# stevenmiller888/mlx-audio

Measured on AMD Instinct MI355X. Metric: audio-sec/sec (xRT), Kokoro-82M batch=32 fixed 128-phoneme utterances per GPU, higher is better.
Workload: dtype bf16; 1 GPU; Kokoro-82M bf16, batch=32/GPU fixed 128-phoneme utterances (T=130, F=650, 390000 samples = 16.25 s each), utterance-sharded over 1 GPU(s); global_batch=32, parallelism=utterance-shard x1, 2 batches in flight per GPU

## Files before the change

include/kokoro_hip.h:

```cpp
#ifndef KOKORO_HIP_H
#define KOKORO_HIP_H

#include <stddef.h>
#include <stdint.h>

#ifdef __cplusplus
extern "C" {
#endif

#define KK_ABI_VERSION 2
#define KK_ABI_MINOR 14

enum { KK_DTYPE_F32 = 0, KK_DTYPE_BF16 = 1, KK_DTYPE_I32 = 2, KK_DTYPE_F16 = 3 };
enum { KK_NOISE_ZERO = 0, KK_NOISE_INJECTED = 1, KK_NOISE_PHILOX = 2 };

typedef struct kk_model kk_model;
typedef struct kk_context kk_context;

typedef struct kk_config {
  int32_t n_token, hidden_dim, style_dim, n_layer, max_dur, text_encoder_kernel_size;
  int32_t plbert_hidden, plbert_heads, plbert_intermediate, plbert_max_pos, plbert_layers, plbert_embedding;
  int32_t decoder_hidden;
  int32_t upsample_initial_channel;
  int32_t n_upsamples;
// ... 56 lines not shown
int kk_op_adain(void* stream, int B, const void* x, int ldx, int L_rows, const int32_t* len, int C, const float* gamma_beta, int gbs,
                int act, float slope, const float* alpha, int pool, const float* pool_w, const float* pool_b, void* out, int ldo, int Cpad,
                int Lout_rows, float* scratch, size_t scratch_floats, int dtype, int fast);
int kk_op_layernorm(void* stream, int B, const void* x, int ldx, const void* res, int ldr, int L_rows, const int32_t* len, int C,
                    const float* w, const float* b, const float* gamma_beta, int gbs, float eps, int act, float slope, void* out, int ldo,
                    int dtype);
int kk_op_lstm(void* stream, int B, const float* xproj, const float* whT, int H, int L_rows, const int32_t* len, void* out, int ldo,
               int dtype);
int kk_op_linear_rows(void* stream, int B, const void* x_bf16, long long xbs, int ldx, int rows, const int32_t* len, const void* w_bf16, int N, int K,
                      const float* bias, int act, void* pack_scratch, void* out_bf16, long long obs, int ldo);
int kk_op_lstm_bf16(void* stream, int B, const float* xproj, const void* wh_bf16, int L_rows, const int32_t* len, void* out, int ldo,
                    int dtype);
int kk_op_attention(void* stream, int B, const void* qkv, int ld, int T_rows, const int32_t* len, int heads, void* out, int ldo, int dtype);
int kk_op_source_stft(void* stream, int B, const float* f0, int L2_rows, const int32_t* len2, const float* lin_w9, float lin_b,
                      int noise_mode, const float* noise, uint64_t seed, float* phase_scratch, float* har_source, void* har, int ldhar,
                      int dtype);
int kk_op_istft_head(void* stream, int B, const void* x, int ldx, int Tf_rows, const int32_t* len_frames, float* wav, int dtype, int fast);
int kk_op_pack_head_w(void* stream, const void* w_bf16, void* w_frag);
int kk_op_conv_post_istft(void* stream, int B, const void* x, int ldx, int Tf_rows, const int32_t* len_frames, const void* w_frag,
                          const float* bias, float in_slope, float* wav, void* cp_out, int cp_ld);

int kk_mxfp8_bytes(int rows, int K, size_t* q_bytes, size_t* s_bytes);
int kk_mxfp8_pack_weight(const float* w_host, int N, int K, int group, uint8_t* q_host, uint8_t* s_host);
int kk_op_linear_mxfp8(void* stream, const void* x_bf16, int ldx, int M, int rows_per_item, const int32_t* len, int K, const void* wq,
                       const void* ws, int N, const float* bias, int act, void* aq, void* as, void* out_bf16, int ldo);

int kk_debug_info(kk_context* cx, const char* name, int64_t* rows, int64_t* channels);
int kk_debug_fetch(kk_context* cx, void* stream, const char* name, float* dst);
int kk_debug_override(kk_context* cx, const char* name, const float* src);
void kk_debug_clear(kk_context* cx);
int kk_op_pack_w_frag(void* stream, const void* w_bf16, void* w_frag, int Kw, int CoutP, int CinP);
void kk_debug_set_op_wfrag(const void* w_frag);
void kk_debug_set_op_variant(int v);
void kk_debug_set_op_post_slope(float slope);
void kk_debug_force_generic(kk_context* cx, int flags);

int kk_profile_begin(kk_context* cx, int max_launches);
int kk_profile_end(kk_context* cx, int ncls, double* ms, double* flops, double* bytes, int64_t* count);

typedef struct kk_mimi kk_mimi;

typedef struct kk_mimi_config {
  int32_t dim, nq, bins, qdim, num_heads, num_layers, dim_feedforward, nfilters;
  int32_t n_ratios, ratios[8];
  int32_t ksize, residual_ksize, last_ksize, upsample_stride, compress;
  float rope_base;
  int32_t compute_dtype;
} kk_mimi_config;

int kk_mimi_create(const kk_mimi_config* cfg, kk_mimi** out);
void kk_mimi_destroy(kk_mimi* m);
int kk_mimi_load_tensor(kk_mimi* m, const char* name, const int64_t* shape, int ndim, const float* data);
int kk_mimi_finalize(kk_mimi* m, void* stream);
int64_t kk_mimi_samples_per_frame(const kk_mimi* m);
size_t kk_mimi_workspace_bytes(kk_mimi* m, int B, int Nf);
int kk_mimi_decode(kk_mimi* m, void* stream, int B, int Nf, const int32_t* codes, void* workspace, size_t workspace_bytes, float* pcm_out);
int kk_mimi_encode_frames(const kk_mimi* m, int N);
size_t kk_mimi_encode_workspace_bytes(kk_mimi* m, int B, int N);
int kk_mimi_encode(kk_mimi* m, void* stream, int B, int N, const float* pcm, void* workspace, size_t workspace_bytes, int32_t* codes_out);
typedef struct kk_mimi_stream kk_mimi_stream;
int kk_mimi_stream_create(kk_mimi* m, int max_batch, int max_frames, kk_mimi_stream** out);
int kk_mimi_stream_create_chunked(kk_mimi* m, int encoder, int max_batch, int max_frames, int chunk_frames, kk_mimi_stream** out);
void kk_mimi_stream_destroy(kk_mimi_stream* s);
int kk_mimi_stream_reset(kk_mimi_stream* s);
int kk_mimi_stream_frames(const kk_mimi_stream* s);
int kk_mimi_stream_chunk_frames(const kk_mimi_stream* s);
// ... 169 lines not shown
```

mlx-audio_amd/_lib.py:

```python
from __future__ import annotations

import ctypes as C
import os

_HERE = os.path.dirname(os.path.abspath(__file__))
LIB_PATH = os.path.join(_HERE, "libkokoro_hip.so")

KK_F32, KK_BF16, KK_I32, KK_F16 = 0, 1, 2, 3
CSM_WEIGHTS = {0: "f32", 1: "bf16", 2: "q8", 3: "q4"}
CSM_WEIGHTS_MIXED, CSM_WEIGHTS_DEQUANTIZED = 0x100, 0x200
NOISE_ZERO, NOISE_INJECTED, NOISE_PHILOX = 0, 1, 2
ACT_NONE, ACT_LRELU, ACT_GELU, ACT_SNAKE = 0, 1, 2, 3
KK_PCM_F32, KK_PCM_S16LE, KK_PCM_MULAW, KK_PCM_ALAW = 0, 1, 2, 3


class KKConfig(C.Structure):
    _fields_ = [
        ("n_token", C.c_int32), ("hidden_dim", C.c_int32), ("style_dim", C.c_int32), ("n_layer", C.c_int32),
        ("max_dur", C.c_int32), ("text_encoder_kernel_size", C.c_int32),
        ("plbert_hidden", C.c_int32), ("plbert_heads", C.c_int32), ("plbert_intermediate", C.c_int32),
        ("plbert_max_pos", C.c_int32), ("plbert_layers", C.c_int32), ("plbert_embedding", C.c_int32),
        ("decoder_hidden", C.c_int32), ("upsample_initial_channel", C.c_int32), ("n_upsamples", C.c_int32),
        ("upsample_rates", C.c_int32 * 4), ("upsample_kernel_sizes", C.c_int32 * 4),
        ("n_resblock_kernels", C.c_int32), ("resblock_kernel_sizes", C.c_int32 * 4),
# ... 153 lines not shown
    "kk_resampler_destroy": (None, [_vp]),
    "kk_resampler_set_row": (_i, [_vp, _vp, _i, _i, _i, _vp, _i]),
    "kk_resampler_step": (_i, [_vp, _vp, _vp, C.c_longlong, _vp, _vp, _vp, C.c_longlong, _vp]),
    "kk_resampler_block_outputs": (_i, []),
    "kk_op_resample": (_i, [_vp, _vp, _i, _i, _i, _vp, _i, _vp]),
    "kk_resampler_set_row_fmt": (_i, [_vp, _vp, _i, _i, _i, _vp, _i, _i, _i]),
    "kk_resampler_step_fmt": (_i, [_vp, _vp, _vp, C.c_longlong, _vp, _vp, _vp, C.c_longlong, _vp]),
    "kk_pcm_convert_rows": (_i, [_vp, _i, _vp, C.c_longlong, _vp, _vp, C.c_longlong, _vp, _vp]),
    "kk_op_pcm_convert": (_i, [_vp, _vp, _i, _vp, _i, _i]),
    "kk_vad_create": (_i, [_i, C.POINTER(_vp)]),
    "kk_vad_destroy": (None, [_vp]),
    "kk_vad_set_row": (_i, [_vp, _vp, _i, _i, _f, _i]),
    "kk_vad_step": (_i, [_vp, _vp, _vp, C.c_longlong, _vp, _vp, _vp, C.c_longlong]),
    "kk_op_vad": (_i, [_vp, _vp, _i, _i, _f, _i, _vp, _vp]),
    "kk_vad_ring_create": (_i, [_i, C.POINTER(_vp)]),
    "kk_vad_ring_destroy": (None, [_vp]),
    "kk_vad_ring_set_row": (_i, [_vp, _vp, _i, _i, _f, _i, C.c_longlong, C.c_longlong]),
    "kk_vad_ring_step": (_i, [_vp, _vp, _vp, C.c_longlong, _vp, _vp, _vp, _vp, _vp, C.c_longlong]),
    "kk_ring_write_rows": (_i, [_vp, _i, _vp, C.c_longlong, _vp, C.c_longlong, C.c_longlong, _vp, _vp]),
    "kk_ring_read_rows": (_i, [_vp, _i, _vp, C.c_longlong, C.c_longlong, _vp, C.c_longlong, _vp, _vp, _vp]),
    "kk_op_log_mel": (_i, [_vp, _i, _vp, C.c_longlong, _vp, _i, _i, _vp, _vp, _vp, _vp, _vp, _i]),
    "kk_op_attention_long": (_i, [_vp, _i, _vp, _i, _i, _i, _i, _vp, _i]),
    "kk_whisper_create": (_i, [C.POINTER(KKWhisperConfig), C.POINTER(_vp)]),
    "kk_whisper_destroy": (None, [_vp]),
    "kk_whisper_load_tensor": (_i, [_vp, C.c_char_p, C.POINTER(C.c_int64), _i, _vp]),
    "kk_whisper_finalize": (_i, [_vp, _vp]),
    "kk_whisper_encode_workspace_bytes": (_sz, [_vp, _i]),
    "kk_whisper_encode": (_i, [_vp, _vp, _i, _vp, _vp, _sz, _vp]),
    "kk_mimi_debug_info": (_i, [_vp, C.c_char_p, C.POINTER(C.c_int64), C.POINTER(C.c_int64)]),
    "kk_mimi_debug_fetch": (_i, [_vp, _vp, C.c_char_p, _vp]),
    "kk_debug_set_op_wfrag": (None, [_vp]),
    "kk_debug_set_op_variant": (None, [_i]),
    "kk_debug_set_op_post_slope": (None, [_f]),
    "kk_set_graph_mode": (_i, [_vp, _i]),
    "kk_set_quantization": (_i, [_vp, _i, _i]),
    "kk_quantized_layers": (_i, [_vp]),
    "kk_mxfp8_bytes": (_i, [_i, _i, C.POINTER(_sz), C.POINTER(_sz)]),
    "kk_mxfp8_pack_weight": (_i, [_vp, _i, _i, _i, _vp, _vp]),
    "kk_op_linear_mxfp8": (_i, [_vp, _vp, _i, _i, _i, _vp, _i, _vp, _vp, _i, _vp, _i, _vp, _vp, _vp, _i]),
    "kk_profile_begin": (_i, [_vp, _i]),
    "kk_profile_end": (_i, [_vp, _i, C.POINTER(C.c_double), C.POINTER(C.c_double), C.POINTER(C.c_double), C.POINTER(C.c_int64)]),
}

_lib = None


class KokoroHipError(RuntimeError):
    pass


def load():
    global _lib
    if _lib is not None:
        return _lib
    path = os.environ.get("KK_HIP_LIB", LIB_PATH)
    if not os.path.exists(path):
        raise KokoroHipError(
            f"{path} not found: build it with `python mlx-audio_amd/build.py` (hipcc, gfx950). "
            "The Kokoro hot path has no CPU or PyTorch fallback."
        )
    try:
        import torch
    except ImportError:
        pass
    lib = C.CDLL(path)
    for name, (res, args) in SIGNATURES.items():
# ... 14 lines not shown
```

mlx-audio_amd/csrc/kk_conv_mfma4.hip:

```cpp
#include <stdlib.h>

#include "kk_common.h"
#include "kk_kernels.h"
#include "kk_conv_mfma_shared.h"

#define TR_NOW() 0ull
#define TR_ADD(slot, v) do { } while (0)
namespace {
typedef __bf16 bf16x2 __attribute__((ext_vector_type(2)));

typedef __bf16 bf16x8 __attribute__((ext_vector_type(8)));
typedef float f32x4 __attribute__((ext_vector_type(4)));

constexpr int BN = 128, CK = 64;
constexpr int XLD = 80;
constexpr int MAX_HALO = 50;
constexpr int CLD = BN;

constexpr int PS_BYTES = 2 * 3 * CK * 4;

template <int BM>
struct Geo {
  static constexpr int XROWS = BM + MAX_HALO;
  static constexpr int XS_BYTES = XROWS * XLD * 2;
  static constexpr int MAIN_BYTES = XS_BYTES + PS_BYTES;
  static constexpr int RPP = BM / 2;
  static constexpr int EPI_BYTES = RPP * CLD * 4;
  static constexpr int LDS_BYTES = MAIN_BYTES > EPI_BYTES ? MAIN_BYTES : EPI_BYTES;
  static constexpr int XREG = (XROWS * 8 + 255) / 256;
};


union U16 {
  uint4 u;
  bf16_t h[8];
};
union U32x8 {
  uint4 u[2];
  float f[8];
};

template <typename TO, int WM, int NRM>
__global__ __launch_bounds__(256, 2) __attribute__((amdgpu_waves_per_eu(2, 2))) void conv_mfma4_kernel(KKMfmaArgs a) {
  constexpr int BM = 2 * WM, MI16 = WM / 16;
  constexpr bool ACC16 = true;
  using G = Geo<BM>;
  constexpr int XREG = G::XREG;
  extern __shared__ __attribute__((aligned(16))) unsigned char smem[];
  bf16_t* Xs = (bf16_t*)smem;
  float* Ps = (float*)(smem + G::XS_BYTES);
  float* Cs = (float*)smem;

  const int tid = threadIdx.x, lane = tid & 63, wave = tid >> 6;
  const int wr = wave >> 1, wc = wave & 1;
  const int nphase = a.mode == KK_CONVT ? a.stride : 1;
  int bx, by, bz;
  {
    const int gx = gridDim.x, gy = gridDim.y, total = gx * gy * gridDim.z;
    int lid = blockIdx.x + gx * (blockIdx.y + gy * blockIdx.z);
    const int per = total / 8, rem = total - per * 8;
    const int xcd = lid & 7, idx = lid >> 3;
    lid = xcd * per + (xcd < rem ? xcd : rem) + idx;
    by = lid % gy;
    const int t = lid / gy;
    bx = t % gx;
    bz = t / gx;
  }
  const int b = bz / nphase, phase = bz - b * nphase;
  const int q0 = bx * BM, n0 = by * BN;
  const int Lin = kk_len(a.lin, b), Lout = kk_len(a.lout, b);

  int ntaps, off0, dstep, widx0, wstep;
  if (a.mode == KK_CONV) {
    ntaps = a.Kw; off0 = -a.pad; dstep = a.dil; widx0 = 0; wstep = 1;
  } else {
    const int k0 = (phase + a.pad) % a.stride;
    ntaps = (a.Kw - k0 + a.stride - 1) / a.stride;
    off0 = (phase + a.pad - k0) / a.stride; dstep = -1; widx0 = k0; wstep = a.stride;
  }
  const int min_off = dstep >= 0 ? off0 : off0 + (ntaps - 1) * dstep;
  const int halo = (ntaps - 1) * (dstep >= 0 ? dstep : -dstep);
  const int xrows = BM + halo;

  const int op_first = a.mode == KK_CONV ? q0 : phase + a.stride * q0;
  const bool tile_live = op_first < Lout;

  const unsigned long long tr0 = TR_NOW();
  unsigned long long tr_sx = 0, tr_sw = 0;
  (void)tr0; (void)tr_sx; (void)tr_sw;
  f32x4 acc[MI16][4];
#pragma unroll
  for (int i = 0; i < MI16; ++i)
#pragma unroll
    for (int j = 0; j < 4; ++j) acc[i][j] = f32x4{0.f, 0.f, 0.f, 0.f};

  if (tile_live) {
    const bf16_t* xb = a.x + (long long)b * a.xbs;
    const int nchunk = a.CinP / CK;
    const int nit = nchunk * ntaps;
    const int lin_hi = Lin > 0 ? Lin - 1 : 0;
    const int cin_real = a.Cin > 0 ? a.Cin : a.CinP;

#define KK_STG(name) name
#define KK_STG_XS Xs
#include "kk_conv_mfma_stage.h"
    uint4 q00, q01, q02, q03, q10, q11, q12, q13;
    const int nb = by;
    auto frag_ptr = [&](int it) __attribute__((always_inline)) -> const uint4* {
      const int chunk = it / ntaps, tap = it - chunk * ntaps;
      const long long blk = ((long long)(widx0 + tap * wstep) * (a.CoutP / BN) + nb) * nchunk + chunk;
      return (const uint4*)a.wf + blk * 1024 + (wc * 2) * 4 * 64 + lane;
    };
    load_x(0);
    {
      const uint4* fp = frag_ptr(0);
      q00 = fp[0 * 64]; q01 = fp[1 * 64]; q02 = fp[2 * 64]; q03 = fp[3 * 64];
      q10 = fp[4 * 64]; q11 = fp[5 * 64]; q12 = fp[6 * 64]; q13 = fp[7 * 64];
      asm volatile("" ::: "memory");
    }
    store_p(0);
    __syncthreads();
    store_x(0);
    __syncthreads();

    const int arow = wr * WM + (lane & 15);
    const int kofs = 8 * (lane >> 4);

    for (int it = 0; it < nit; ++it) {
      const int chunk = it / ntaps, tap = it - chunk * ntaps;
      const bool last_tap = tap == ntaps - 1;
      if (tap == 0 && chunk + 1 < nchunk) load_x(chunk + 1);
      const uint4* fn = frag_ptr(it + 1 < nit ? it + 1 : it);

      const int shift = (off0 + tap * dstep) - min_off;
      const bf16_t* xa = Xs + (arow + shift) * XLD + kofs;
      KK_MFMA_ITER(q00, q01, q02, q03, q10, q11, q12, q13)
      asm volatile("" ::: "memory");
      if (it + 1 < nit) {
        if (tap == 0 && chunk + 1 < nchunk) store_p(chunk + 1);
        if (last_tap) {
          __syncthreads();
          store_x(chunk + 1);
          __syncthreads();
        }
      }
    }
    __syncthreads();
  }

#include "kk_conv_mfma_epilogue.h"
}

template <int XR>
struct GeoWK {
  static constexpr int SROWS = XR == 7 ? 224 : 192 + MAX_HALO;
  static constexpr int SLAB = SROWS * XLD;
  static constexpr int XS_BYTES = 2 * SLAB * 2;
  static constexpr int MAIN_BYTES = XS_BYTES + PS_BYTES;
  static constexpr int RPP = 96;
  static constexpr int EPI_BYTES = RPP * CLD * 4;
  static constexpr int LDS_BYTES = MAIN_BYTES > EPI_BYTES ? MAIN_BYTES : EPI_BYTES;
};

template <int NRM, int XR>
__global__ __launch_bounds__(256, 2) __attribute__((amdgpu_waves_per_eu(2, 2))) void conv_mfma4_wholek_kernel(KKMfmaArgs a) {
  using TO = bf16_t;
  constexpr int WM = 96, BM = 2 * WM, MI16 = WM / 16, XREG = XR;
  constexpr bool ACC16 = true;
  using G = GeoWK<XR>;
  extern __shared__ __attribute__((aligned(16))) unsigned char smem[];
  bf16_t* Xs = (bf16_t*)smem;
  float* Ps = (float*)(smem + G::XS_BYTES);
  float* Cs = (float*)smem;

  const int tid = threadIdx.x, lane = tid & 63, wave = tid >> 6;
  const int wr = wave >> 1, wc = wave & 1;
  constexpr int nphase = 1, phase = 0;
  int bx, by, b;
  {
    const int gx = gridDim.x, gy = gridDim.y, total = gx * gy * gridDim.z;
    int lid = blockIdx.x + gx * (blockIdx.y + gy * blockIdx.z);
    const int per = total / 8, rem = total - per * 8;
    const int xcd = lid & 7, idx = lid >> 3;
    lid = xcd * per + (xcd < rem ? xcd : rem) + idx;
    by = lid % gy;
    const int t = lid / gy;
    bx = t % gx;
    b = t / gx;
  }
  const int q0 = bx * BM, n0 = by * BN;
  const int Lin = kk_len(a.lin, b), Lout = kk_len(a.lout, b);
  const int ntaps = a.Kw, off0 = -a.pad, dstep = a.dil, min_off = off0;
  const int xrows = BM + (ntaps - 1) * dstep;
  const bool tile_live = q0 < Lout;

  const unsigned long long tr0 = TR_NOW();
  (void)tr0;
  f32x4 acc[MI16][4];
#pragma unroll
  for (int i = 0; i < MI16; ++i)
#pragma unroll
    for (int j = 0; j < 4; ++j) acc[i][j] = f32x4{0.f, 0.f, 0.f, 0.f};

  if (tile_live) {
    const bf16_t* xb = a.x + (long long)b * a.xbs;
    const int nit = 2 * ntaps;
    const int lin_hi = Lin > 0 ? Lin - 1 : 0;
    const int cin_real = a.Cin > 0 ? a.Cin : a.CinP;

#define KK_STG(name) name##_s0
#define KK_STG_XS Xs
#include "kk_conv_mfma_stage.h"
#define KK_STG(name) name##_s1
#define KK_STG_XS (Xs + G::SLAB)
#include "kk_conv_mfma_stage.h"
    uint4 q00, q01, q02, q03, q10, q11, q12, q13;
    auto frag_ptr = [&](int it) __attribute__((always_inline)) -> const uint4* {
      const int chunk = it >= ntaps ? 1 : 0, tap = it - chunk * ntaps;
      const long long blk = ((long long)tap * (a.CoutP / BN) + by) * 2 + chunk;
      return (const uint4*)a.wf + blk * 1024 + (wc * 2) * 4 * 64 + lane;
    };
    load_x_s0(0);
    load_x_s1(1);
    {
      const uint4* fp = frag_ptr(0);
      q00 = fp[0 * 64]; q01 = fp[1 * 64]; q02 = fp[2 * 64]; q03 = fp[3 * 64];
      q10 = fp[4 * 64]; q11 = fp[5 * 64]; q12 = fp[6 * 64]; q13 = fp[7 * 64];
      asm volatile("" ::: "memory");
    }
    store_p_s0(0);
    store_p_s1(1);
    __syncthreads();
    store_x_s0(0);
    store_x_s1(1);
    __syncthreads();

    const int arow = wr * WM + (lane & 15);
    const int kofs = 8 * (lane >> 4);
    for (int it = 0; it + 1 < nit; ++it) {
      const int chunk = it >= ntaps ? 1 : 0, tap = it - chunk * ntaps;
      const uint4* fn = frag_ptr(it + 1);
      const bf16_t* xa = Xs + chunk * G::SLAB + (arow + tap * dstep) * XLD + kofs;
      KK_MFMA_ITER(q00, q01, q02, q03, q10, q11, q12, q13)
      asm volatile("" ::: "memory");
    }
    {
      const bf16_t* xa = Xs + G::SLAB + (arow + (ntaps - 1) * dstep) * XLD + kofs;
      KK_MFMA_ITER_LAST(q00, q01, q02, q03, q10, q11, q12, q13)
      asm volatile("" ::: "memory");
    }
    __syncthreads();
  }

#include "kk_conv_mfma_epilogue.h"
}

template <int NRM, int XR>
int launch_wholek(const KKMfmaArgs& a, int B, hipStream_t st) {
  using G = GeoWK<XR>;
  static KKDevOnce attr_once;
  if (attr_once.first()) {
    (void)hipFuncSetAttribute((const void*)conv_mfma4_wholek_kernel<NRM, XR>, hipFuncAttributeMaxDynamicSharedMemorySize, G::LDS_BYTES);
    attr_once.done();
  }
  dim3 grid(kk_cdiv(a.Q, 192), a.CoutP / BN, B);
  hipLaunchKernelGGL((conv_mfma4_wholek_kernel<NRM, XR>), grid, dim3(256), G::LDS_BYTES, st, a);
  KK_CHECK_LAUNCH();
  return 0;
}

template <typename TO, int WM, int NRM>
int launch_one(const KKMfmaArgs& a, int B, hipStream_t st) {
  using G = Geo<2 * WM>;
  static KKDevOnce attr_once;
  if (attr_once.first()) {
    (void)hipFuncSetAttribute((const void*)conv_mfma4_kernel<TO, WM, NRM>, hipFuncAttributeMaxDynamicSharedMemorySize, G::LDS_BYTES);
    attr_once.done();
  }
  const int nphase = a.mode == KK_CONVT ? a.stride : 1;
  dim3 grid(kk_cdiv(a.Q, 2 * WM), a.CoutP / BN, B * nphase);
  hipLaunchKernelGGL((conv_mfma4_kernel<TO, WM, NRM>), grid, dim3(256), G::LDS_BYTES, st, a);
  KK_CHECK_LAUNCH();
  return 0;
}

__global__ __launch_bounds__(256) void pack_w_frag_kernel(const bf16_t* w, bf16_t* wf, int Kw, int CoutP, int CinP) {
  const long long n = (long long)Kw * CoutP * CinP;
// ... 39 lines not shown
```

mlx-audio_amd/csrc/kk_model.hip:

```cpp
#include <math.h>
#include <stdio.h>
#include <string.h>

#include <algorithm>
#include <functional>
#include <map>
#include <string>
#include <vector>

#include "../../include/kokoro_hip.h"
#include "kk_common.h"
#include "kk_kernels.h"
#include "kk_host.h"

static thread_local std::string g_err;
static const void* g_op_wfrag = nullptr;
static float g_op_post_slope = 0.f;
static int g_op_variant = 4;

int kk_fail(const char* msg) {
  g_err = msg ? msg : "unknown error";
  return -1;
}
extern "C" const char* kk_last_error(void) { return g_err.c_str(); }
extern "C" int kk_abi_version(void) { return KK_ABI_VERSION; }
extern "C" int kk_abi_minor(void) { return KK_ABI_MINOR; }

namespace {

struct ConvW {
  size_t w_off = 0, b_off = 0;
  bool has_bias = false;
  int Cin = 0, Cout = 0, Kw = 0, ldw = 0;
  const float* w = nullptr;
  const float* b = nullptr;
  bool mfma = false;
  size_t wb_off = 0, wf_off = 0;
  int CinP = 0, CoutP = 0, Cout8 = 0;
  const bf16_t* wb = nullptr;
  const bf16_t* wf = nullptr;
  size_t wl_off = 0;
  const bf16_t* wl = nullptr;
  bool fp8 = false;
  size_t q8_off = 0, s8_off = 0;
  const uint4* q8 = nullptr;
  const unsigned char* s8 = nullptr;
};
struct LstmW {
  ConvW in;
  ArenaVec whT;
  int H = 0;
// ... 1511 lines not shown
                            int ldo, int Lout_rows, const int32_t* lout, int in_dtype, int out_dtype) {
  KKConvArgs a;
  memset(&a, 0, sizeof a);
  a.x = x; a.xbs = (long long)Lin_rows * ldx; a.ldx = ldx; a.w = w_packed; a.ldw = ldw; a.bias = bias;
  a.out = out; a.obs = (long long)Lout_rows * ldo; a.ldo = ldo;
  a.res = res; a.rbs = (long long)Lout_rows * ldr; a.ldr = ldr;
  a.Cin = Cin; a.Cout = Cout; a.Kw = Kw; a.mode = transposed ? KK_CONVT : KK_CONV; a.stride = stride; a.pad = pad; a.dil = dil;
  a.in_shift = in_shift; a.Q = transposed ? kk_cdiv(Lout_rows, stride) : Lout_rows; a.Lo_rows = Lout_rows;
  a.lin = KKLen{lin, lin ? 1 : 0, lin ? 0 : Lin_rows};
  a.lout = KKLen{lout, lout ? 1 : 0, lout ? 0 : Lout_rows};
  a.in_slope = in_slope; a.scale = scale; a.accumulate = accumulate; a.act = act; a.act_slope = act_slope;
  return kk_launch_conv_generic(a, B, in_dtype, out_dtype, (hipStream_t)stream);
}

extern "C" int kk_op_conv1d_bf16(void* stream, int B, const void* x, int ldx, int Lin_rows, const int32_t* lin, const void* w_bf16, int CinP,
                                 int CoutP, const float* bias, int Cout, int Kw, int transposed, int stride, int pad, int dil, int in_shift,
                                 float in_slope, int act, float act_slope, const void* res, int ldr, float scale, int accumulate, void* out,
                                 int ldo, int Lout_rows, const int32_t* lout, int out_dtype) {
  KKMfmaArgs g;
  memset(&g, 0, sizeof g);
  g.x = (const bf16_t*)x; g.xbs = (long long)Lin_rows * ldx; g.ldx = ldx; g.w = (const bf16_t*)w_bf16; g.CinP = CinP; g.CoutP = CoutP; g.bias = bias;
  g.out = out; g.obs = (long long)Lout_rows * ldo; g.ldo = ldo; g.res = res; g.rbs = (long long)Lout_rows * ldr; g.ldr = ldr;
  g.Cout = Cout; g.Kw = Kw; g.mode = transposed ? KK_CONVT : KK_CONV; g.stride = stride; g.pad = pad; g.dil = dil; g.in_shift = in_shift;
  g.Q = transposed ? kk_cdiv(Lout_rows, stride) : Lout_rows; g.Lo_rows = Lout_rows;
  g.lin = KKLen{lin, lin ? 1 : 0, lin ? 0 : Lin_rows};
  g.lout = KKLen{lout, lout ? 1 : 0, lout ? 0 : Lout_rows};
  g.in_slope = in_slope; g.scale = scale; g.accumulate = accumulate; g.act = act; g.act_slope = act_slope;
  if (!kk_mfma_eligible(CinP, Cout, Kw, g.mode, stride, dil)) return kk_fail("kk_op_conv1d_bf16: shape not eligible for the MFMA kernel");
  if (g_op_wfrag && out_dtype == KK_BF16) {
    g.wf = (const bf16_t*)g_op_wfrag;
    g.post_slope = g_op_post_slope;
    if (g_op_variant == 5 && kk_mfma5_eligible(g, out_dtype)) return kk_launch_conv_mfma5(g, B, out_dtype, (hipStream_t)stream);
    g.slabwise = g_op_variant == 40;
    return kk_launch_conv_mfma4(g, B, out_dtype, (hipStream_t)stream);
  }
  return kk_launch_conv_mfma(g, B, out_dtype, (hipStream_t)stream);
}

extern "C" int kk_op_conv1d_bf16_fused(void* stream, int B, const void* x, int ldx, int L_rows, const int32_t* len, const void* w_bf16, int CinP,
                                       int CoutP, const float* bias, int Cin, int Cout, int Kw, int pad, int dil, const float* nrm_a,
                                       const float* nrm_b, int nrm_stride, int nrm_act, float nrm_slope, const float* nrm_alpha,
                                       const void* res, int ldr, float scale, void* out, int ldo, float* stat_part, int* stat_ntiles_out) {
  KKMfmaArgs g;
  memset(&g, 0, sizeof g);
  g.x = (const bf16_t*)x; g.xbs = (long long)L_rows * ldx; g.ldx = ldx; g.w = (const bf16_t*)w_bf16; g.CinP = CinP; g.Cin = Cin; g.CoutP = CoutP; g.bias = bias;
  g.out = out; g.obs = (long long)L_rows * ldo; g.ldo = ldo; g.res = res; g.rbs = (long long)L_rows * ldr; g.ldr = ldr;
  g.Cout = Cout; g.Kw = Kw; g.mode = KK_CONV; g.stride = 1; g.pad = pad; g.dil = dil; g.Q = L_rows; g.Lo_rows = L_rows;
  g.lin = KKLen{len, len ? 1 : 0, len ? 0 : L_rows};
  g.lout = g.lin;
  g.in_slope = 1.f; g.scale = scale;
  g.nrm_a = nrm_a; g.nrm_b = nrm_b; g.nrm_stride = nrm_stride; g.nrm_act = nrm_act; g.nrm_slope = nrm_slope; g.nrm_alpha = nrm_alpha; g.nrm_C = Cin;
  g.stat_part = stat_part;
  g.stat_ntiles = kk_cdiv(L_rows, KK_MFMA_TILE_ROWS);
  if (stat_ntiles_out) *stat_ntiles_out = g.stat_ntiles;
  if (!kk_mfma_eligible(CinP, Cout, Kw, KK_CONV, 1, dil)) return kk_fail("kk_op_conv1d_bf16_fused: shape not eligible for the MFMA kernel");
  if (g_op_wfrag) {
    g.wf = (const bf16_t*)g_op_wfrag;
    g.post_slope = g_op_post_slope;
    if (g_op_variant == 5 && kk_mfma5_eligible(g, KK_BF16)) return kk_launch_conv_mfma5(g, B, KK_BF16, (hipStream_t)stream);
    g.slabwise = g_op_variant == 40;
    return kk_launch_conv_mfma4(g, B, KK_BF16, (hipStream_t)stream);
  }
  return kk_launch_conv_mfma(g, B, KK_BF16, (hipStream_t)stream);
}

extern "C" int kk_op_adain(void* stream, int B, const void* x, int ldx, int L_rows, const int32_t* len, int C, const float* gamma_beta,
                           int gbs, int act, float slope, const float* alpha, int pool, const float* pool_w, const float* pool_b, void* out,
// ... 150 lines not shown
  if (!m || !m->finalized) return -1;
  const ConvW* set[] = {&m->map_in, &m->qkv, &m->att_dense, &m->ffn, &m->ffn_out, &m->bert_encoder};
  int n = 0;
  for (const ConvW* c : set) n += c->fp8 ? 1 : 0;
  return n;
}

extern "C" int kk_mxfp8_bytes(int rows, int K, size_t* q_bytes, size_t* s_bytes) {
  if (rows <= 0 || K <= 0 || K % 64 || !q_bytes || !s_bytes) return kk_fail("kk_mxfp8_bytes: bad argument");
  *q_bytes = kk_mxfp8_q_bytes(rows, K);
  *s_bytes = kk_mxfp8_s_bytes(rows, K);
  return 0;
}
extern "C" int kk_mxfp8_pack_weight(const float* w_host, int N, int K, int group, uint8_t* q_host, uint8_t* s_host) {
  if (!w_host || !q_host || !s_host) return kk_fail("kk_mxfp8_pack_weight: null argument");
  return kk_mxfp8_pack_weight_host(w_host, N, K, group, q_host, s_host);
}
extern "C" int kk_op_linear_mxfp8(void* stream, const void* x_bf16, int ldx, int M, int rows_per_item, const int32_t* len, int K,
                                  const void* wq, const void* ws, int N, const float* bias, int act, void* aq, void* as, void* out_bf16,
                                  int ldo) {
  if (!x_bf16 || !wq || !ws || !aq || !as || !out_bf16) return kk_fail("kk_op_linear_mxfp8: null argument");
  KK_TRY(kk_launch_mxfp8_quant_rows(x_bf16, ldx, M, K, aq, as, (hipStream_t)stream));
  KKFp8Args f;
  memset(&f, 0, sizeof f);
  f.aq = (const uint4*)aq; f.as = (const unsigned char*)as; f.wq = (const uint4*)wq; f.ws = (const unsigned char*)ws;
  f.M = M; f.N = N; f.K = K; f.bias = bias; f.out = (bf16_t*)out_bf16; f.ldo = ldo; f.rows_per_item = rows_per_item;
  f.lout = KKLen{len, len ? 1 : 0, len ? 0 : rows_per_item};
  f.act = act;
  return kk_launch_linear_mxfp8(f, (hipStream_t)stream);
}
extern "C" void kk_debug_set_op_wfrag(const void* w_frag) { g_op_wfrag = w_frag; }
extern "C" void kk_debug_set_op_post_slope(float slope) { g_op_post_slope = slope; }
extern "C" void kk_debug_set_op_variant(int v) { g_op_variant = (v == 5 || v == 40) ? v : 4; }
extern "C" int kk_op_pack_w_frag(void* stream, const void* w_bf16, void* w_frag, int Kw, int CoutP, int CinP) {
  return kk_launch_pack_w_frag(w_bf16, w_frag, Kw, CoutP, CinP, (hipStream_t)stream);
}
extern "C" void kk_debug_clear(kk_context* cx) {
  if (!cx) return;
  cx->dbg_over.clear();
  cx->dbg.map.clear();
}

extern "C" int kk_profile_begin(kk_context* cx, int max_launches) {
  if (!cx || max_launches <= 0) return kk_fail("kk_profile_begin: bad argument");
  while ((int)cx->prof_ev.size() < 2 * max_launches) {
    hipEvent_t e;
    if (hipEventCreate(&e) != hipSuccess) return kk_fail("kk_profile_begin: hipEventCreate failed");
    cx->prof_ev.push_back(e);
  }
  cx->prof_rec.clear();
  cx->prof_on = true;
  return 0;
}
extern "C" int kk_profile_end(kk_context* cx, int ncls, double* ms, double* flops, double* bytes, int64_t* count) {
  if (!cx || !ms || !flops || !bytes || !count) return kk_fail("kk_profile_end: null argument");
  for (int i = 0; i < ncls; ++i) { ms[i] = 0; flops[i] = 0; bytes[i] = 0; count[i] = 0; }
  cx->prof_on = false;
  for (size_t i = 0; i < cx->prof_rec.size(); ++i) {
    if (hipEventSynchronize(cx->prof_ev[2 * i + 1]) != hipSuccess) return kk_fail("kk_profile_end: event sync failed");
    float t = 0.f;
    if (hipEventElapsedTime(&t, cx->prof_ev[2 * i], cx->prof_ev[2 * i + 1]) != hipSuccess) return kk_fail("kk_profile_end: elapsed failed");
    const auto& r = cx->prof_rec[i];
    if (r.cls >= 0 && r.cls < ncls) { ms[r.cls] += t; flops[r.cls] += r.flops; bytes[r.cls] += r.bytes; count[r.cls] += 1; }
  }
  cx->prof_rec.clear();
  return 0;
// ... 2 lines not shown
```

Baseline: 15440 audio-sec/sec.

## Replace block-wide conv epilogue with per-wave LDS staging and prefetched residuals

The mfma4 conv kernels now stage accumulators through small per-wave LDS regions (double-buffered in the whole-K kernel) instead of a block-wide epilogue buffer. This removes block-level barriers from the epilogue and keeps the whole-K kernel's LDS footprint unchanged. Residual rows are prefetched before the output passes, and channel statistics are reduced across waves through LDS. Debug hooks for stats and flat-row launches, plus optional cycle tracing, are added; the new epilogue path adds register pressure from the prefetch and kept values.

```diff
diff --git a/include/kokoro_hip.h b/include/kokoro_hip.h
--- a/include/kokoro_hip.h
+++ b/include/kokoro_hip.h
@@ -112,6 +112,8 @@
 int kk_op_pack_w_frag(void* stream, const void* w_bf16, void* w_frag, int Kw, int CoutP, int CinP);
 void kk_debug_set_op_wfrag(const void* w_frag);
 void kk_debug_set_op_variant(int v);
+void kk_debug_set_op_stats(float* stat_part);
+void kk_debug_set_op_flat(int on);
 void kk_debug_set_op_post_slope(float slope);
 void kk_debug_force_generic(kk_context* cx, int flags);
 
diff --git a/mlx-audio_amd/_lib.py b/mlx-audio_amd/_lib.py
--- a/mlx-audio_amd/_lib.py
+++ b/mlx-audio_amd/_lib.py
@@ -209,6 +209,8 @@
     "kk_debug_set_op_wfrag": (None, [_vp]),
     "kk_debug_set_op_variant": (None, [_i]),
     "kk_debug_set_op_post_slope": (None, [_f]),
+    "kk_debug_set_op_stats": (None, [_vp]),
+    "kk_debug_set_op_flat": (None, [_i]),
     "kk_set_graph_mode": (_i, [_vp, _i]),
     "kk_set_quantization": (_i, [_vp, _i, _i]),
     "kk_quantized_layers": (_i, [_vp]),
diff --git a/mlx-audio_amd/csrc/kk_conv_mfma4.hip b/mlx-audio_amd/csrc/kk_conv_mfma4.hip
--- a/mlx-audio_amd/csrc/kk_conv_mfma4.hip
+++ b/mlx-audio_amd/csrc/kk_conv_mfma4.hip
@@ -4,8 +4,30 @@
 #include "kk_kernels.h"
 #include "kk_conv_mfma_shared.h"
 
+#ifdef KK_MFMA_TRACE
+__device__ unsigned long long kk_mfma4_trace_acc[1024][8];
+#define TR_NOW() (__builtin_readcyclecounter())
+#define TR_ADD(slot, v) \
+  do { if (threadIdx.x == 0) atomicAdd(&kk_mfma4_trace_acc[(blockIdx.x + 37 * blockIdx.z) & 1023][slot], (unsigned long long)(v)); } while (0)
+extern "C" int kk_debug_mfma4_trace(unsigned long long* out8, int reset) {
+  static unsigned long long h[1024][8];
+  if (out8) {
+    if (hipMemcpyFromSymbol(h, HIP_SYMBOL(kk_mfma4_trace_acc), sizeof(h)) != hipSuccess) return -1;
+    for (int k = 0; k < 8; ++k) out8[k] = 0;
+    for (int r = 0; r < 1024; ++r)
+      for (int k = 0; k < 8; ++k) out8[k] += h[r][k];
+  }
+  if (reset) {
+    for (int r = 0; r < 1024; ++r)
+      for (int k = 0; k < 8; ++k) h[r][k] = 0;
+    if (hipMemcpyToSymbol(HIP_SYMBOL(kk_mfma4_trace_acc), h, sizeof(h)) != hipSuccess) return -1;
+  }
+  return 0;
+}
+#else
 #define TR_NOW() 0ull
 #define TR_ADD(slot, v) do { } while (0)
+#endif
 namespace {
 typedef __bf16 bf16x2 __attribute__((ext_vector_type(2)));
 
@@ -15,7 +37,8 @@
 constexpr int BN = 128, CK = 64;
 constexpr int XLD = 80;
 constexpr int MAX_HALO = 50;
-constexpr int CLD = BN;
+constexpr int EPI_ROWS = 32, EPI_LD = 68;
+constexpr int epi_waves_bytes(int nbuf) { return 4 * nbuf * EPI_ROWS * EPI_LD * 4; }
 
 constexpr int PS_BYTES = 2 * 3 * CK * 4;
 
@@ -24,9 +47,8 @@
   static constexpr int XROWS = BM + MAX_HALO;
   static constexpr int XS_BYTES = XROWS * XLD * 2;
   static constexpr int MAIN_BYTES = XS_BYTES + PS_BYTES;
-  static constexpr int RPP = BM / 2;
-  static constexpr int EPI_BYTES = RPP * CLD * 4;
-  static constexpr int LDS_BYTES = MAIN_BYTES > EPI_BYTES ? MAIN_BYTES : EPI_BYTES;
+  static constexpr int EPR = EPI_ROWS, EPLD = EPI_LD, EPBUF = 1;
+  static constexpr int LDS_BYTES = MAIN_BYTES > epi_waves_bytes(EPBUF) ? MAIN_BYTES : epi_waves_bytes(EPBUF);
   static constexpr int XREG = (XROWS * 8 + 255) / 256;
 };
 
@@ -43,13 +65,11 @@
 template <typename TO, int WM, int NRM>
 __global__ __launch_bounds__(256, 2) __attribute__((amdgpu_waves_per_eu(2, 2))) void conv_mfma4_kernel(KKMfmaArgs a) {
   constexpr int BM = 2 * WM, MI16 = WM / 16;
-  constexpr bool ACC16 = true;
   using G = Geo<BM>;
   constexpr int XREG = G::XREG;
   extern __shared__ __attribute__((aligned(16))) unsigned char smem[];
   bf16_t* Xs = (bf16_t*)smem;
   float* Ps = (float*)(smem + G::XS_BYTES);
-  float* Cs = (float*)smem;
 
   const int tid = threadIdx.x, lane = tid & 63, wave = tid >> 6;
   const int wr = wave >> 1, wc = wave & 1;
@@ -86,8 +106,7 @@
   const bool tile_live = op_first < Lout;
 
   const unsigned long long tr0 = TR_NOW();
-  unsigned long long tr_sx = 0, tr_sw = 0;
-  (void)tr0; (void)tr_sx; (void)tr_sw;
+  (void)tr0;
   f32x4 acc[MI16][4];
 #pragma unroll
   for (int i = 0; i < MI16; ++i)
@@ -122,6 +141,9 @@
     __syncthreads();
     store_x(0);
     __syncthreads();
+    const unsigned long long tr1 = TR_NOW();
+    (void)tr1;
+    TR_ADD(0, tr1 - tr0);
 
     const int arow = wr * WM + (lane & 15);
     const int kofs = 8 * (lane >> 4);
@@ -146,9 +168,10 @@
       }
     }
     __syncthreads();
-  }
-
-#include "kk_conv_mfma_epilogue.h"
+    TR_ADD(1, TR_NOW() - tr1);
+  }
+
+#include "kk_conv_mfma_epilogue_waves.h"
 }
 
 template <int XR>
@@ -157,21 +180,19 @@
   static constexpr int SLAB = SROWS * XLD;
   static constexpr int XS_BYTES = 2 * SLAB * 2;
   static constexpr int MAIN_BYTES = XS_BYTES + PS_BYTES;
-  static constexpr int RPP = 96;
-  static constexpr int EPI_BYTES = RPP * CLD * 4;
-  static constexpr int LDS_BYTES = MAIN_BYTES > EPI_BYTES ? MAIN_BYTES : EPI_BYTES;
+  static constexpr int EPR = EPI_ROWS, EPLD = EPI_LD, EPBUF = 2;
+  static constexpr int LDS_BYTES = MAIN_BYTES > epi_waves_bytes(EPBUF) ? MAIN_BYTES : epi_waves_bytes(EPBUF);
+  static_assert(LDS_BYTES == MAIN_BYTES, "the epilogue regions must not grow the whole-K kernel's LDS");
 };
 
 template <int NRM, int XR>
 __global__ __launch_bounds__(256, 2) __attribute__((amdgpu_waves_per_eu(2, 2))) void conv_mfma4_wholek_kernel(KKMfmaArgs a) {
   using TO = bf16_t;
   constexpr int WM = 96, BM = 2 * WM, MI16 = WM / 16, XREG = XR;
-  constexpr bool ACC16 = true;
   using G = GeoWK<XR>;
   extern __shared__ __attribute__((aligned(16))) unsigned char smem[];
   bf16_t* Xs = (bf16_t*)smem;
   float* Ps = (float*)(smem + G::XS_BYTES);
-  float* Cs = (float*)smem;
 
   const int tid = threadIdx.x, lane = tid & 63, wave = tid >> 6;
   const int wr = wave >> 1, wc = wave & 1;
@@ -234,6 +255,9 @@
     store_x_s0(0);
     store_x_s1(1);
     __syncthreads();
+    const unsigned long long tr1 = TR_NOW();
+    (void)tr1;
+    TR_ADD(0, tr1 - tr0);
 
     const int arow = wr * WM + (lane & 15);
     const int kofs = 8 * (lane >> 4);
@@ -250,9 +274,10 @@
       asm volatile("" ::: "memory");
     }
     __syncthreads();
-  }
-
-#include "kk_conv_mfma_epilogue.h"
+    TR_ADD(1, TR_NOW() - tr1);
+  }
+
+#include "kk_conv_mfma_epilogue_waves.h"
 }
 
 template <int NRM, int XR>
diff --git a/mlx-audio_amd/csrc/kk_conv_mfma_epilogue_waves.h b/mlx-audio_amd/csrc/kk_conv_mfma_epilogue_waves.h
--- /dev/null
+++ b/mlx-audio_amd/csrc/kk_conv_mfma_epilogue_waves.h
@@ -0,0 +1,235 @@
+  static_assert(sizeof(TO) == 2 && WM % G::EPR == 0 && G::EPR % 16 == 0, "per-wave epilogue: bf16 outputs, 16 x 16 blocks");
+  TO* ob = (TO*)a.out + (long long)b * a.obs;
+  const TO* rb = a.res ? (const TO*)a.res + (long long)b * a.rbs : nullptr;
+  const int lrow = 4 * (lane >> 5) + ((0xD728 >> (2 * ((lane >> 2) & 7))) & 3), lpc = ((lane >> 1) & 4) | (lane & 3);
+  const int n = n0 + wc * 64 + lpc * 8;
+  const int nc = n < a.Cout ? n : 0;
+  const int lo_hi = a.Lo_rows - 1;
+  const bool tile_full = tile_live && !a.flat_T && (a.mode == KK_CONV ? q0 + BM - 1 : phase + a.stride * (q0 + BM - 1)) < Lout;
+  v2f bias2[4];
+#pragma unroll
+  for (int k = 0; k < 4; ++k)
+    bias2[k] = a.bias ? v2f{a.bias[n + 2 * k], a.bias[n + 2 * k + 1]} : v2f{0.f, 0.f};
+  const v2f scale2 = {a.scale, a.scale}, act_slope2 = {a.act_slope, a.act_slope};
+  v2f cs[2][4], cq[2][4];
+#pragma unroll
+  for (int c = 0; c < 2; ++c)
+#pragma unroll
+    for (int k = 0; k < 4; ++k) cs[c][k] = cq[c][k] = v2f{0.f, 0.f};
+  v2f keep[(WM / G::EPR) * (G::EPR / 8)][4];
+  unsigned keep_ok = 0;
+  const bool stat_now = a.stat_part && wr == 0;
+
+  constexpr int EPR = G::EPR, EPLD = G::EPLD, NPASS = WM / EPR, TASKS = EPR / 8;
+  constexpr int NBUF = G::EPBUF;
+  float* Cw = (float*)smem + wave * (NBUF * EPR * EPLD);
+  auto dump = [&](int pass) __attribute__((always_inline)) {
+    float* cw = Cw + (pass % NBUF) * (EPR * EPLD);
+#pragma unroll
+    for (int mi = 0; mi < EPR / 16; ++mi)
+#pragma unroll
+      for (int ni = 0; ni < 4; ++ni)
+#pragma unroll
+        for (int r = 0; r < 4; ++r) cw[(mi * 16 + 4 * (lane >> 4) + r) * EPLD + ni * 16 + (lane & 15)] = acc[pass * (EPR / 16) + mi][ni][r];
+  };
+  const int qw = q0 + wr * WM + lrow;
+  uint4 rpre[NPASS * TASKS];
+  if (rb) {
+#pragma unroll
+    for (int j = 0; j < NPASS * TASKS; ++j) {
+      const int q = qw + j * 8;
+      const int op = a.mode == KK_CONV ? q : phase + a.stride * q;
+      const int opc = op < 0 ? 0 : (op > lo_hi ? lo_hi : op);
+      rpre[j] = *(const uint4*)(rb + (long long)opc * a.ldr + nc);
+    }
+    asm volatile("" ::: "memory");
+  }
+  TR_ADD(2, TR_NOW() - tr0);
+#pragma unroll
+  for (int pass = 0; pass < NPASS; ++pass) {
+    int opv[TASKS];
+    bool wr_ok[TASKS], live[TASKS];
+    uint4 rold[TASKS];
+#pragma unroll
+    for (int i = 0; i < TASKS; ++i) {
+      const int q = qw + (pass * TASKS + i) * 8;
+      const int op = a.mode == KK_CONV ? q : phase + a.stride * q;
+      opv[i] = op < 0 ? 0 : (op > lo_hi ? lo_hi : op);
+      wr_ok[i] = q < a.Q && op < a.Lo_rows && n < a.Cout;
+      live[i] = tile_live && op < Lout;
+      if (a.flat_T) {
+        const int bb = opv[i] / a.flat_T;
+        live[i] = live[i] && (opv[i] - bb * a.flat_T) < kk_len(a.flat_len, bb);
+      }
+    }
+    if (a.accumulate) {
+#pragma unroll
+      for (int i = 0; i < TASKS; ++i) rold[i] = *(const uint4*)(ob + (long long)opv[i] * a.ldo + nc);
+      asm volatile("" ::: "memory");
+    }
+    float4 cb[TASKS][2];
+    if (tile_live) {
+      if (pass == 0 || NBUF == 1) {
+        __builtin_amdgcn_fence(__ATOMIC_ACQ_REL, "wavefront");
+        __builtin_amdgcn_wave_barrier();
+        dump(pass);
+      }
+      __builtin_amdgcn_fence(__ATOMIC_ACQ_REL, "wavefront");
+      __builtin_amdgcn_wave_barrier();
+      const float* cp = Cw + (pass % NBUF) * (EPR * EPLD) + lrow * EPLD + lpc * 8;
+#pragma unroll
+      for (int i = 0; i < TASKS; ++i) {
+        cb[i][0] = *(const float4*)(cp + i * 8 * EPLD);
+        cb[i][1] = *(const float4*)(cp + i * 8 * EPLD + 4);
+      }
+      if (NBUF == 2 && pass + 1 < NPASS) {
+        __builtin_amdgcn_fence(__ATOMIC_ACQ_REL, "wavefront");
+        __builtin_amdgcn_wave_barrier();
+        dump(pass + 1);
+      }
+    }
+    if (pass == 0) TR_ADD(6, TR_NOW() - tr0);
+#pragma unroll
+    for (int i = 0; i < TASKS; ++i) {
+      v2f v[4];
+      if (tile_live) {
+        const float4 c0 = cb[i][0], c1 = cb[i][1];
+        v[0] = v2f{c0.x, c0.y}; v[1] = v2f{c0.z, c0.w}; v[2] = v2f{c1.x, c1.y}; v[3] = v2f{c1.z, c1.w};
+      } else {
+#pragma unroll
+        for (int k = 0; k < 4; ++k) v[k] = v2f{0.f, 0.f};
+      }
+#pragma unroll
+      for (int k = 0; k < 4; ++k) v[k] += bias2[k];
+      if (a.act == KK_ACT_LRELU) {
+#pragma unroll
+        for (int k = 0; k < 4; ++k) {
+          const v2f m = v[k] * act_slope2;
+          v[k].x = v[k].x > 0.f ? v[k].x : m.x;
+          v[k].y = v[k].y > 0.f ? v[k].y : m.y;
+        }
+      } else if (a.act == KK_ACT_GELU) {
+#pragma unroll
+        for (int k = 0; k < 4; ++k) {
+          v[k].x = gelu_exact(v[k].x);
+          v[k].y = gelu_exact(v[k].y);
+        }
+      } else if (NRM == 0 && a.act == KK_ACT_GELU_TANH) {
+#pragma unroll
+        for (int k = 0; k < 4; ++k) {
+          v[k].x = 0.5f * v[k].x * (1.0f + tanhf(0.7978845608028654f * (v[k].x + 0.044715f * (v[k].x * v[k].x * v[k].x))));
+          v[k].y = 0.5f * v[k].y * (1.0f + tanhf(0.7978845608028654f * (v[k].y + 0.044715f * (v[k].y * v[k].y * v[k].y))));
+        }
+      }
+      if (rb) {
+        const uint4 rr = rpre[pass * TASKS + i];
+        const unsigned w4[4] = {rr.x, rr.y, rr.z, rr.w};
+#pragma unroll
+        for (int k = 0; k < 4; ++k) v[k] += v2f{__uint_as_float(w4[k] << 16), __uint_as_float(w4[k] & 0xFFFF0000u)};
+      }
+      if (a.scale != 1.0f) {
+#pragma unroll
+        for (int k = 0; k < 4; ++k) v[k] *= scale2;
+      }
+      if (a.accumulate) {
+        const unsigned w4[4] = {rold[i].x, rold[i].y, rold[i].z, rold[i].w};
+#pragma unroll
+        for (int k = 0; k < 4; ++k) v[k] += v2f{__uint_as_float(w4[k] << 16), __uint_as_float(w4[k] & 0xFFFF0000u)};
+      }
+      if (a.post_slope != 0.f && a.post_slope != 1.0f) {
+#pragma unroll
+        for (int k = 0; k < 4; ++k) {
+          const float mx = v[k].x * a.post_slope, my = v[k].y * a.post_slope;
+          v[k].x = v[k].x > mx ? v[k].x : mx;
+          v[k].y = v[k].y > my ? v[k].y : my;
+        }
+      }
+      if (!tile_full && !live[i]) {
+#pragma unroll
+        for (int k = 0; k < 4; ++k) v[k] = v2f{0.f, 0.f};
+      }
+      unsigned w4[4];
+#pragma unroll
+      for (int k = 0; k < 4; ++k) {
+        const bf16x2 pk = {(bf16_t)v[k].x, (bf16_t)v[k].y};
+        w4[k] = __builtin_bit_cast(unsigned, pk);
+      }
+      if (wr_ok[i]) *(uint4*)(ob + (long long)opv[i] * a.ldo + n) = make_uint4(w4[0], w4[1], w4[2], w4[3]);
+#pragma unroll
+      for (int k = 0; k < 4; ++k) keep[pass * TASKS + i][k] = v[k];
+      keep_ok |= (wr_ok[i] ? 1u : 0u) << (pass * TASKS + i);
+      if (stat_now && wr_ok[i]) {
+#pragma unroll
+        for (int k = 0; k < 4; ++k) {
+          cs[i & 1][k] += v[k];
+          cq[i & 1][k] = fma2(v[k], v[k], cq[i & 1][k]);
+        }
+      }
+    }
+    if (pass == 0) TR_ADD(7, TR_NOW() - tr0);
+  }
+  TR_ADD(4, TR_NOW() - tr0);
+  TR_ADD(5, 1);
+  if (a.stat_part) {
+    constexpr int NT = NPASS * TASKS, REG = NBUF * EPR * EPLD;
+    static_assert(TASKS % 2 == 0 && 16 * 2 * 64 <= REG, "chains: rows 8 apart alternate between two chains; [16 chains][2][64 columns] fit a wave region");
+    float* xch = (float*)smem + wc * REG;
+    float* fin = (float*)smem + (2 + wc) * REG;
+    if (wr == 0) {
+      __builtin_amdgcn_fence(__ATOMIC_ACQ_REL, "wavefront");
+      __builtin_amdgcn_wave_barrier();
+#pragma unroll
+      for (int c = 0; c < 2; ++c) {
+        float4* xp = (float4*)(xch + ((lrow + 8 * c) * 2) * 64 + lpc * 8);
+        xp[0] = make_float4(cs[c][0].x, cs[c][0].y, cs[c][1].x, cs[c][1].y);
+        xp[1] = make_float4(cs[c][2].x, cs[c][2].y, cs[c][3].x, cs[c][3].y);
+        xp[16] = make_float4(cq[c][0].x, cq[c][0].y, cq[c][1].x, cq[c][1].y);
+        xp[17] = make_float4(cq[c][2].x, cq[c][2].y, cq[c][3].x, cq[c][3].y);
+      }
+    }
+    __syncthreads();
+    if (wr == 1) {
+#pragma unroll
+      for (int c = 0; c < 2; ++c) {
+        const float4* xp = (const float4*)(xch + ((lrow + 8 * c) * 2) * 64 + lpc * 8);
+        const float4 s0 = xp[0], s1 = xp[1], q0v = xp[16], q1v = xp[17];
+        cs[c][0] = v2f{s0.x, s0.y}; cs[c][1] = v2f{s0.z, s0.w}; cs[c][2] = v2f{s1.x, s1.y}; cs[c][3] = v2f{s1.z, s1.w};
+        cq[c][0] = v2f{q0v.x, q0v.y}; cq[c][1] = v2f{q0v.z, q0v.w}; cq[c][2] = v2f{q1v.x, q1v.y}; cq[c][3] = v2f{q1v.z, q1v.w};
+      }
+#pragma unroll
+      for (int j = 0; j < NT; ++j) {
+        if ((keep_ok >> j) & 1u) {
+#pragma unroll
+          for (int k = 0; k < 4; ++k) {
+            cs[j & 1][k] += keep[j][k];
+            cq[j & 1][k] = fma2(keep[j][k], keep[j][k], cq[j & 1][k]);
+          }
+        }
+      }
+      __builtin_amdgcn_fence(__ATOMIC_ACQ_REL, "wavefront");
+      __builtin_amdgcn_wave_barrier();
+#pragma unroll
+      for (int c = 0; c < 2; ++c) {
+        float4* xp = (float4*)(fin + ((lrow + 8 * c) * 2) * 64 + lpc * 8);
+        xp[0] = make_float4(cs[c][0].x, cs[c][0].y, cs[c][1].x, cs[c][1].y);
+        xp[1] = make_float4(cs[c][2].x, cs[c][2].y, cs[c][3].x, cs[c][3].y);
+        xp[16] = make_float4(cq[c][0].x, cq[c][0].y, cq[c][1].x, cq[c][1].y);
+        xp[17] = make_float4(cq[c][2].x, cq[c][2].y, cq[c][3].x, cq[c][3].y);
+      }
+      __builtin_amdgcn_fence(__ATOMIC_ACQ_REL, "wavefront");
+      __builtin_amdgcn_wave_barrier();
+      const int col = n0 + wc * 64 + lane, tile = bx * nphase + phase;
+#pragma unroll
+      for (int which = 0; which < 2; ++which) {
+        float t[4];
+#pragma unroll
+        for (int w = 0; w < 4; ++w) {
+          const float* fp = fin + ((4 * w) * 2 + which) * 64 + lane;
+          t[w] = (fp[0] + fp[128]) + (fp[256] + fp[384]);
+        }
+        const float v = ((t[0] + t[1]) + t[2]) + t[3];
+        if (col < a.Cout) a.stat_part[(((long long)b * a.stat_ntiles + tile) * 2 + which) * a.Cout + col] = v;
+      }
+    }
+    TR_ADD(3, TR_NOW() - tr0);
+  }
diff --git a/mlx-audio_amd/csrc/kk_model.hip b/mlx-audio_amd/csrc/kk_model.hip
--- a/mlx-audio_amd/csrc/kk_model.hip
+++ b/mlx-audio_amd/csrc/kk_model.hip
@@ -17,6 +17,8 @@
 static const void* g_op_wfrag = nullptr;
 static float g_op_post_slope = 0.f;
 static int g_op_variant = 4;
+static float* g_op_stat_part = nullptr;
+static int g_op_flat = 0;
 
 int kk_fail(const char* msg) {
   g_err = msg ? msg : "unknown error";
@@ -1594,7 +1596,23 @@
     g.post_slope = g_op_post_slope;
     if (g_op_variant == 5 && kk_mfma5_eligible(g, out_dtype)) return kk_launch_conv_mfma5(g, B, out_dtype, (hipStream_t)stream);
     g.slabwise = g_op_variant == 40;
-    return kk_launch_conv_mfma4(g, B, out_dtype, (hipStream_t)stream);
+    if (g_op_stat_part) {
+      g.stat_part = g_op_stat_part;
+      g.stat_ntiles = kk_cdiv(g.Q, KK_MFMA_TILE_ROWS) * (transposed ? stride : 1);
+    }
+    int Bl = B;
+    if (g_op_flat) {
+      if (B < 2 || Kw != 1 || transposed || stride != 1 || pad != 0 || dil != 1 || in_shift != 0 || g_op_stat_part || Lin_rows != Lout_rows)
+        return kk_fail("kk_op_conv1d_bf16: launch not eligible for flat rows");
+      g.flat_T = Lout_rows;
+      g.flat_len = g.lout;
+      g.Q = B * Lout_rows;
+      g.Lo_rows = B * Lout_rows;
+      g.lin = KKLen{nullptr, 0, g.Q};
+      g.lout = KKLen{nullptr, 0, g.Q};
+      Bl = 1;
+    }
+    return kk_launch_conv_mfma4(g, Bl, out_dtype, (hipStream_t)stream);
   }
   return kk_launch_conv_mfma(g, B, out_dtype, (hipStream_t)stream);
 }
@@ -1811,6 +1829,8 @@
 extern "C" void kk_debug_set_op_wfrag(const void* w_frag) { g_op_wfrag = w_frag; }
 extern "C" void kk_debug_set_op_post_slope(float slope) { g_op_post_slope = slope; }
 extern "C" void kk_debug_set_op_variant(int v) { g_op_variant = (v == 5 || v == 40) ? v : 4; }
+extern "C" void kk_debug_set_op_stats(float* stat_part) { g_op_stat_part = stat_part; }
+extern "C" void kk_debug_set_op_flat(int on) { g_op_flat = on; }
 extern "C" int kk_op_pack_w_frag(void* stream, const void* w_bf16, void* w_frag, int Kw, int CoutP, int CinP) {
   return kk_launch_pack_w_frag(w_bf16, w_frag, Kw, CoutP, CinP, (hipStream_t)stream);
 }
```

Result: no change. 15560 audio-sec/sec, median of 6 (+0.8%).
